# BrandonHanx/TextReID

Hardware: AMD Instinct MI355X
Metric: image-text pairs/sec (train), CLIP-RN50 + BiGRU MoCo step, bs128/GPU (higher is better)
Workload: dtype f32; 1 GPU; configs[1]: CLIP-RN50 + GRU, bs128/GPU, 384x128 images, 64-token captions, MoCo queue 8192, fp32, 1xMI355X; random-init weights, synthetic inputs resident in HBM; global_batch=128, parallelism=dp1, optimizer=Adam (fused multi-tensor), step_launch=eager launches, four streams (chosen by the probe over the recorded step)

## Files before the change

### textreid_amd/csrc/gemm_p16.hip

```cpp

#include <algorithm>
#include <mutex>
#include <type_traits>

#include "split_common.h"

namespace trid {

constexpr int P16_BK = 32;

constexpr int p16_lds_bytes(int BM, int BN, int NW, int STAGES) {
    const int st = STAGES * (BM + BN) * 128;
    return (NW == 12 && BM * BN * 4 > st) ? BM * BN * 4 : st;
}

template <int N>
__device__ __forceinline__ void wait_vmcnt() {
    asm volatile("s_waitcnt vmcnt(%0)" ::"n"(N) : "memory");
}

__device__ __forceinline__ void dma16(const __amdgpu_buffer_rsrc_t& rs, uint4* lds_base, unsigned voffset, unsigned soffset) {
    typedef __attribute__((address_space(3))) void* lds_ptr;
    __builtin_amdgcn_raw_ptr_buffer_load_lds(rs, (lds_ptr)lds_base, 16, voffset, soffset, 0, 0);
}
// ... 622 lines not shown
            if (bnb) {
                b_mu = *reinterpret_cast<const float4*>(bb.mean + col);
                b_is = *reinterpret_cast<const float4*>(bb.invstd + col);
                b_sc = *reinterpret_cast<const float4*>(bb.scale + col);
                b_sh = *reinterpret_cast<const float4*>(bb.shift + col);
            }
#pragma unroll
            for (int ps = 0; ps < BM / RG; ++ps) {
                const int rl = ps * RG + rg, row = m0 + rl;
                if (row >= p.M || col >= p.N) continue;
                float4 v = *reinterpret_cast<const float4*>(Ct + rl * BN + 4 * c4);
                const long long at = (long long)row * p.ldc + col;
                float4 yv = make_float4(0.f, 0.f, 0.f, 0.f);
                if (bnb) yv = *reinterpret_cast<const float4*>(bb.y + (long long)row * p.N + col);
                if (!pre) {
                    v.x += bv4.x; v.y += bv4.y; v.z += bv4.z; v.w += bv4.w;
                    if (p.accumulate) {
                        float4 u;
                        if (p.c_fmt == 2) {
                            const uint2 ub = *reinterpret_cast<const uint2*>(Cb + at);
                            u = make_float4(__builtin_bit_cast(float, ub.x << 16), __builtin_bit_cast(float, ub.x & 0xffff0000u),
                                            __builtin_bit_cast(float, ub.y << 16), __builtin_bit_cast(float, ub.y & 0xffff0000u));
                        } else {
                            u = *reinterpret_cast<const float4*>(C + at);
                        }
                        if (p.cmask != nullptr) {
                            const long long qi = at >> 2;
                            const ulonglong2* mq = reinterpret_cast<const ulonglong2*>(p.cmask + (qi >> 6) * 4);
                            const ulonglong2 m01 = mq[0], m23 = mq[1];
                            const int bit = (int)(qi & 63);
                            u.x = ((m01.x >> bit) & 1ull) ? u.x : 0.f; u.y = ((m01.y >> bit) & 1ull) ? u.y : 0.f;
                            u.z = ((m23.x >> bit) & 1ull) ? u.z : 0.f; u.w = ((m23.y >> bit) & 1ull) ? u.w : 0.f;
                        }
                        v.x += u.x; v.y += u.y; v.z += u.z; v.w += u.w;
                    }
                    if (p.res != nullptr) {
                        const float4 rr = *reinterpret_cast<const float4*>(p.res + (long long)row * p.ldres + col);
                        v.x += rr.x; v.y += rr.y; v.z += rr.z; v.w += rr.w;
                    }
                    if (p.relu) { v.x = fmaxf(v.x, 0.f); v.y = fmaxf(v.y, 0.f); v.z = fmaxf(v.z, 0.f); v.w = fmaxf(v.w, 0.f); }
                }
                if (p.c_fmt == 2) *reinterpret_cast<uint2*>(Cb + at) = make_uint2(cvt_pk_bf16(v.x, v.y), cvt_pk_bf16(v.z, v.w));
                else *reinterpret_cast<float4*>(C + at) = v;
                if (bnb) {
                    const float4 xh = make_float4((yv.x - b_mu.x) * b_is.x, (yv.y - b_mu.y) * b_is.y, (yv.z - b_mu.z) * b_is.z, (yv.w - b_mu.w) * b_is.w);
                    float4 g = v;
                    if (bb.relu == 1) {
                        g.x = fmaf(yv.x, b_sc.x, b_sh.x) > 0.f ? g.x : 0.f; g.y = fmaf(yv.y, b_sc.y, b_sh.y) > 0.f ? g.y : 0.f;
                        g.z = fmaf(yv.z, b_sc.z, b_sh.z) > 0.f ? g.z : 0.f; g.w = fmaf(yv.w, b_sc.w, b_sh.w) > 0.f ? g.w : 0.f;
                    } else if (bb.relu == 2) {
                        const long long qi = ((long long)row * p.N + col) >> 2;
                        const ulonglong2* mq = reinterpret_cast<const ulonglong2*>(bb.mask + (qi >> 6) * 4);
                        const ulonglong2 m01 = mq[0], m23 = mq[1];
                        const int bit = (int)(qi & 63);
                        g.x = ((m01.x >> bit) & 1ull) ? g.x : 0.f; g.y = ((m01.y >> bit) & 1ull) ? g.y : 0.f;
                        g.z = ((m23.x >> bit) & 1ull) ? g.z : 0.f; g.w = ((m23.y >> bit) & 1ull) ? g.w : 0.f;
                    }
                    b_s1.x += g.x; b_s1.y += g.y; b_s1.z += g.z; b_s1.w += g.w;
                    b_s2.x = fmaf(g.x, xh.x, b_s2.x); b_s2.y = fmaf(g.y, xh.y, b_s2.y); b_s2.z = fmaf(g.z, xh.z, b_s2.z); b_s2.w = fmaf(g.w, xh.w, b_s2.w);
                    b_mg.x = fmaxf(b_mg.x, fabsf(g.x)); b_mg.y = fmaxf(b_mg.y, fabsf(g.y)); b_mg.z = fmaxf(b_mg.z, fabsf(g.z)); b_mg.w = fmaxf(b_mg.w, fabsf(g.w));
                    b_mx.x = fmaxf(b_mx.x, fabsf(xh.x)); b_mx.y = fmaxf(b_mx.y, fabsf(xh.y)); b_mx.z = fmaxf(b_mx.z, fabsf(xh.z)); b_mx.w = fmaxf(b_mx.w, fabsf(xh.w));
                }
            }
            if (bb.y != nullptr) {
                __syncthreads();
                float* redf = reinterpret_cast<float*>(smem);
                float* mine = redf + (rg * C4 + c4) * 16;
                *reinterpret_cast<float4*>(mine) = b_s1;
                *reinterpret_cast<float4*>(mine + 4) = b_s2;
                *reinterpret_cast<float4*>(mine + 8) = b_mg;
                *reinterpret_cast<float4*>(mine + 12) = b_mx;
                __syncthreads();
                if (tid < C4 && n0 + 4 * tid < p.N) {
                    float4 s1 = make_float4(0.f, 0.f, 0.f, 0.f), s2 = s1, mg = s1, mx = s1;
                    for (int r = 0; r < RG; ++r) {
                        const float* src = redf + (r * C4 + tid) * 16;
                        const float4 a = *reinterpret_cast<const float4*>(src), b = *reinterpret_cast<const float4*>(src + 4);
                        const float4 c = *reinterpret_cast<const float4*>(src + 8), d = *reinterpret_cast<const float4*>(src + 12);
                        s1.x += a.x; s1.y += a.y; s1.z += a.z; s1.w += a.w;
                        s2.x += b.x; s2.y += b.y; s2.z += b.z; s2.w += b.w;
                        mg.x = fmaxf(mg.x, c.x); mg.y = fmaxf(mg.y, c.y); mg.z = fmaxf(mg.z, c.z); mg.w = fmaxf(mg.w, c.w);
                        mx.x = fmaxf(mx.x, d.x); mx.y = fmaxf(mx.y, d.y); mx.z = fmaxf(mx.z, d.z); mx.w = fmaxf(mx.w, d.w);
                    }
                    const int CQ = p.N >> 2, CW = CQ < 256 ? CQ : 256, S = CQ / CW;
                    const int q = (n0 >> 2) + tid;
                    const long long e = bn_bwd_partial_index(mb * S + q / CW, q % CW, p.mblocks * S, CQ);
                    *reinterpret_cast<float4*>(bb.ws + e) = s1;
                    *reinterpret_cast<float4*>(bb.ws + e + 4) = s2;
                    *reinterpret_cast<float4*>(bb.ws2 + e) = mg;
                    *reinterpret_cast<float4*>(bb.ws2 + e + 4) = mx;
                }
            }
            return;
        }
    }
#pragma unroll
    for (int j = 0; j < TN; ++j) {
        const int col = col_base + 32 * j;
        const float bv = (bias != nullptr && col < p.N) ? bias[col] : 0.f;
#pragma unroll
        for (int i = 0; i < TM; ++i) {
            float oldv[16];
            if (p.accumulate) {
#pragma unroll
                for (int r = 0; r < 16; ++r) {
                    const int row = row_base + i * 32 + (r & 3) + 8 * (r >> 2);
                    const long long at = (long long)row * p.ldc + col;
                    if (row < p.M && col < p.N) {
                        oldv[r] = p.c_fmt == 2 ? __builtin_bit_cast(float, (unsigned)Cb[at] << 16) : C[at];
                        if (p.cmask != nullptr && !((p.cmask[((at >> 2) >> 6) * 4 + (at & 3)] >> ((at >> 2) & 63)) & 1ull)) oldv[r] = 0.f;
                    } else {
                        oldv[r] = 0.f;
                    }
                }
            }
#pragma unroll
            for (int r = 0; r < 16; ++r) {
                const int row = row_base + i * 32 + (r & 3) + 8 * (r >> 2);
                float v = p.alpha * unscale * acc[i][j][r] + bv;
                if (p.accumulate) v += oldv[r];
                if (p.res != nullptr && row < p.M && col < p.N) v += p.res[(long long)row * p.ldres + col];
                if (p.relu) v = fmaxf(v, 0.f);
                if (row < p.M && col < p.N) {
                    const long long at = (long long)row * p.ldc + col;
                    if (p.c_fmt == 2) Cb[at] = (unsigned short)(cvt_pk_bf16(v, 0.f) & 0xffffu);
                    else C[at] = v;
                }
                acc[i][j][r] = p.c_fmt == 2 ? __builtin_bit_cast(float, cvt_pk_bf16(v, 0.f) << 16) : v;
            }
        }
    }

    if (p.stats != nullptr) emit_stats();
}

typedef __fp16 h4v __attribute__((__vector_size__(4 * sizeof(__fp16))));

__device__ __forceinline__ f16x8 tr_frag(const char* lds_addr) {
    typedef __attribute__((address_space(3))) h4v* lp;
    const h4v lo = __builtin_amdgcn_ds_read_tr16_b64_v4f16((lp)(lds_addr));
    const h4v hi = __builtin_amdgcn_ds_read_tr16_b64_v4f16((lp)(lds_addr + 512));
    f16x8 r;
    r[0] = lo[0]; r[1] = lo[1]; r[2] = lo[2]; r[3] = lo[3];
    r[4] = hi[0]; r[5] = hi[1]; r[6] = hi[2]; r[7] = hi[3];
    return r;
}

template <int BMODE, int BM, int STAGES, int PL, int SP = 0>
__global__ __launch_bounds__(512, 4) void gemm_p16_wgrad_kernel(GemmParams p) {
    constexpr int BN = 128, NW = 8, WN = 4, WM = 2;
    constexpr int GC = PL == 2 ? 32 : 64;
    constexpr int PBK = PL == 2 ? 32 : 64;
    constexpr int EB = PL == 2 ? 4 : 2;
    constexpr int CPG = PBK / 8;
    constexpr int TM = BM / (32 * WM);
    constexpr int A_CH = (BM / GC) * CPG, B_CH = (BN / GC) * CPG;
    constexpr int A_PW = (A_CH + NW - 1) / NW, B_PW = B_CH / NW;
    constexpr int PER_TILE = A_PW + B_PW;
    constexpr int GBYTES = PBK * 128;
    constexpr int A_BYTES = (BM / GC) * GBYTES, STAGE_BYTES = A_BYTES + (BN / GC) * GBYTES;
    extern __shared__ __attribute__((aligned(16))) uint4 smem[];
    char* const sbase = reinterpret_cast<char*>(smem);

    const float scaleA = (PL == 2 && p.a_amax != nullptr) ? f16_scale_of(*p.a_amax) : 1.f;
    const float scaleB = (PL == 2 && p.b_amax != nullptr) ? f16_scale_of(*p.b_amax) : 1.f;
    const int tid = threadIdx.x;
    const int lane = tid & 63;
    const int wave = __builtin_amdgcn_readfirstlane(tid >> 6);
    const int wm = wave / WN, wn = wave % WN;

    const uint32_t nwg = (uint32_t)p.mblocks * (uint32_t)p.nblocks;
    uint32_t lid;
    int sz;
    if (p.xcd_split) {
        const uint32_t slot = blockIdx.x >> 3;
        sz = (int)((slot / nwg) * 8 + (blockIdx.x & 7));
        lid = slot % nwg;
        if (sz >= p.splits) return;
    } else {
        lid = xcd_remap(blockIdx.x, nwg);
        sz = blockIdx.z;
    }
    const int mb = lid / p.nblocks, nb = lid % p.nblocks;
    const int m0 = mb * BM, n0 = nb * BN;
    const int k_begin = sz * p.k_chunk;
    const int k_end = min(p.K, k_begin + p.k_chunk);
    const int nk = (k_end - k_begin + PBK - 1) / PBK;
    float* __restrict__ C = p.C + (long long)sz * p.sSplit;

    constexpr unsigned OOB = 0x80000000u;
    const char* A = reinterpret_cast<const char*>(p.A);
    const char* Bp = reinterpret_cast<const char*>(p.B);
    const long long a_ld = p.lda * EB, b_ld = (BMODE == B_CONV ? (long long)p.Cin : p.ldb) * EB;
    const __amdgpu_buffer_rsrc_t rsA = __builtin_amdgcn_make_buffer_rsrc((void*)A, 0, (unsigned)((long long)p.K * a_ld), 0x00020000);
    const char* b_base = (BMODE == B_CONV) ? Bp - (long long)(p.W + 1) * b_ld : Bp;
    const long long b_rows = (BMODE == B_CONV) ? (long long)p.K + 2 * p.W + 2 : p.K;
    const __amdgpu_buffer_rsrc_t rsB = __builtin_amdgcn_make_buffer_rsrc((void*)b_base, 0, (unsigned)(b_rows * b_ld), 0x00020000);

    unsigned voA[A_PW], voB[B_PW];
    int b_pp[B_PW], b_dy[B_PW], b_dx[B_PW];
#pragma unroll
    for (int j = 0; j < A_PW; ++j) {
        const int c = j * NW + wave;
        const int gi = c / CPG, pp = 8 * (c % CPG) + (lane >> 3);
        const int s = (lane & 7) ^ (((pp >> 1) & 1) << 2);
        voA[j] = (c < A_CH && m0 + GC * gi < p.M) ? (unsigned)((long long)pp * a_ld + (m0 + GC * gi) * EB + 16 * s) : OOB;
    }
#pragma unroll
    for (int j = 0; j < B_PW; ++j) {
        const int c = j * NW + wave;
        const int gi = c / CPG, pp = 8 * (c % CPG) + (lane >> 3);
        const int s = (lane & 7) ^ (((pp >> 1) & 1) << 2);
        const int col = n0 + GC * gi;
        b_pp[j] = pp;
        b_dy[j] = b_dx[j] = 0;
        if (BMODE == B_CONV) {
            const int tap = col / p.Cin, c0 = col - tap * p.Cin;
            b_dy[j] = tap / 3 - 1;
            b_dx[j] = tap % 3 - 1;
            voB[j] = col < p.N ? (unsigned)((long long)(pp + (b_dy[j] + 1) * p.W + (b_dx[j] + 1)) * b_ld + c0 * EB + 16 * s) : OOB;
        } else {
            voB[j] = col < p.N ? (unsigned)((long long)pp * b_ld + col * EB + 16 * s) : OOB;
        }
    }

    auto issue = [&](int kt, int stage) {
        char* sA = sbase + stage * STAGE_BYTES;
        char* sB = sA + A_BYTES;
        const int k0 = k_begin + kt * PBK;
        const unsigned soA = (unsigned)((long long)k0 * a_ld), soB = (unsigned)((long long)k0 * b_ld);
#pragma unroll
        for (int j = 0; j < A_PW; ++j) {
            const int c = j * NW + wave;
            if (A_CH % NW != 0 && c >= A_CH) break;
            const unsigned vo = (k0 + 8 * (c % CPG) + (lane >> 3) < k_end) ? voA[j] : OOB;
            dma16(rsA, reinterpret_cast<uint4*>(sA + c * 1024), vo, soA);
        }
#pragma unroll
        for (int j = 0; j < B_PW; ++j) {
            const int c = j * NW + wave;
            unsigned vo = voB[j];
            const int m = k0 + b_pp[j];
            bool ok = m < k_end;
            if (BMODE == B_CONV) {
                const uint32_t q = fdiv((uint32_t)m, p.fdW);
                const int x = m - (int)q * p.W;
                const uint32_t b = fdiv(q, p.fdH);
                const int y = (int)q - (int)b * p.H;
                const int yy = y + b_dy[j], xx = x + b_dx[j];
                ok = ok && yy >= 0 && yy < p.H && xx >= 0 && xx < p.W;
            }
            dma16(rsB, reinterpret_cast<uint4*>(sB + c * 1024), ok ? vo : OOB, soB);
        }
    };

    v16f acc[TM];
#pragma unroll
    for (int i = 0; i < TM; ++i)
#pragma unroll
        for (int r = 0; r < 16; ++r) acc[i][r] = 0.f;

    const int h = (lane >> 4) & 1, r4 = (lane & 15) >> 2, c8 = lane & 3, kh = lane >> 5;
    const int swz = (r4 >> 1) << 2;
    auto frag_off = [&](int sub, int pl, int ks) {
        const int gi = (32 * sub) / GC;
        const int slot = PL == 2 ? (pl * 4 + h * 2 + (c8 >> 1)) : (((sub & 1) * 2 + h) * 2 + (c8 >> 1));
        return gi * GBYTES + (16 * ks + 8 * kh + r4) * 128 + ((slot ^ swz) << 4) + 8 * (c8 & 1);
    };

    auto compute = [&](int stage) {
        const char* sA = sbase + stage * STAGE_BYTES;
        const char* sB = sA + A_BYTES;
        if constexpr (PL == 1) {
#pragma unroll
            for (int ks = 0; ks < 4; ++ks) {
                bf16x8 a[TM], b;
#pragma unroll
                for (int i = 0; i < TM; ++i) a[i] = __builtin_bit_cast(bf16x8, tr_frag(sA + frag_off(wm * TM + i, 0, ks)));
                b = __builtin_bit_cast(bf16x8, tr_frag(sB + frag_off(wn, 0, ks)));
#pragma unroll
                for (int i = 0; i < TM; ++i) acc[i] = __builtin_amdgcn_mfma_f32_32x32x16_bf16(a[i], b, acc[i], 0, 0, 0);
            }
        } else {
#pragma unroll
            for (int ks = 0; ks < 2; ++ks) {
                f16x8 a[2][TM], b[2];
#pragma unroll
                for (int pl = 0; pl < 2; ++pl) {
#pragma unroll
                    for (int i = 0; i < TM; ++i) a[pl][i] = tr_frag(sA + frag_off(wm * TM + i, pl, ks));
                    b[pl] = tr_frag(sB + frag_off(wn, pl, ks));
                }
#pragma unroll
                for (int i = 0; i < TM; ++i) acc[i] = __builtin_amdgcn_mfma_f32_32x32x16_f16(a[0][i], b[1], acc[i], 0, 0, 0);
#pragma unroll
                for (int i = 0; i < TM; ++i) acc[i] = __builtin_amdgcn_mfma_f32_32x32x16_f16(a[1][i], b[0], acc[i], 0, 0, 0);
#pragma unroll
                for (int i = 0; i < TM; ++i) acc[i] = __builtin_amdgcn_mfma_f32_32x32x16_f16(a[0][i], b[0], acc[i], 0, 0, 0);
            }
        }
    };

    const bool wave_live = (m0 + wm * (32 * TM) < p.M) && (n0 + wn * 32 < p.N);
    if constexpr (SP != 0) {
        static_assert(STAGES == 2 && PL == 2, "software pipeline: two stages, P16 operands");
        const v4i_t rsA_s = raw_rsrc(A, (unsigned)((long long)p.K * a_ld)), rsB_s = raw_rsrc(b_base, (unsigned)(b_rows * b_ld));
        const unsigned smem_base = (unsigned)(uintptr_t)(__attribute__((address_space(3))) void*)smem;
        unsigned nvA[A_PW], nvB[B_PW], n_soA = 0, n_soB = 0;
        auto prep = [&](int kt) {
            const int k0 = k_begin + kt * PBK;
            n_soA = (unsigned)((long long)k0 * a_ld);
            n_soB = (unsigned)((long long)k0 * b_ld);
#pragma unroll
            for (int j = 0; j < A_PW; ++j) {
                const int c = j * NW + wave;
                nvA[j] = (k0 + 8 * (c % CPG) + (lane >> 3) < k_end) ? voA[j] : OOB;
            }
#pragma unroll
            for (int j = 0; j < B_PW; ++j) {
                const int m = k0 + b_pp[j];
                bool ok = m < k_end;
                if (BMODE == B_CONV) {
                    const uint32_t q = fdiv((uint32_t)m, p.fdW);
                    const int x = m - (int)q * p.W;
                    const uint32_t b = fdiv(q, p.fdH);
                    const int y = (int)q - (int)b * p.H;
                    const int yy = y + b_dy[j], xx = x + b_dx[j];
                    ok = ok && yy >= 0 && yy < p.H && xx >= 0 && xx < p.W;
                }
                nvB[j] = ok ? voB[j] : OOB;
            }
        };
        auto fire = [&](int stage) {
            const unsigned sA = smem_base + (unsigned)(stage * STAGE_BYTES), sB = sA + A_BYTES;
#pragma unroll
            for (int j = 0; j < A_PW; ++j) {
                const int c = j * NW + wave;
                if (A_CH % NW != 0 && c >= A_CH) break;
                dma16_asm(rsA_s, sA + (unsigned)c * 1024u, nvA[j], n_soA);
            }
#pragma unroll
            for (int j = 0; j < B_PW; ++j) dma16_asm(rsB_s, sB + (unsigned)(j * NW + wave) * 1024u, nvB[j], n_soB);
        };
        f16x8 f0a[2][TM], f0b[2], f1a[2][TM], f1b[2];
        auto rd = [&](int stage, int ks, f16x8 (&fa)[2][TM], f16x8 (&fb)[2]) {
            const char* sA = sbase + stage * STAGE_BYTES;
            const char* sB = sA + A_BYTES;
#pragma unroll
            for (int pl = 0; pl < 2; ++pl) {
#pragma unroll
                for (int i = 0; i < TM; ++i) fa[pl][i] = tr_frag(sA + frag_off(wm * TM + i, pl, ks));
                fb[pl] = tr_frag(sB + frag_off(wn, pl, ks));
            }
        };
        auto mm = [&](const f16x8 (&fa)[2][TM], const f16x8 (&fb)[2]) {
#pragma unroll
            for (int i = 0; i < TM; ++i) acc[i] = __builtin_amdgcn_mfma_f32_32x32x16_f16(fa[0][i], fb[1], acc[i], 0, 0, 0);
#pragma unroll
            for (int i = 0; i < TM; ++i) acc[i] = __builtin_amdgcn_mfma_f32_32x32x16_f16(fa[1][i], fb[0], acc[i], 0, 0, 0);
#pragma unroll
            for (int i = 0; i < TM; ++i) acc[i] = __builtin_amdgcn_mfma_f32_32x32x16_f16(fa[0][i], fb[0], acc[i], 0, 0, 0);
        };
        auto tile = [&](int t, auto stage_c) {
            constexpr int stage = decltype(stage_c)::value;
            asm volatile("s_waitcnt vmcnt(0)" ::: "memory");
            __builtin_amdgcn_s_waitcnt(0x0070);
            __builtin_amdgcn_s_barrier();
            asm volatile("" ::: "memory");
            if (wave_live) rd(stage, 0, f0a, f0b);
            __builtin_amdgcn_sched_barrier(0);
            if (t + 1 < nk) fire(stage ^ 1);
            __builtin_amdgcn_sched_barrier(0);
            if (wave_live) {
                if (t > 0) mm(f1a, f1b);
                __builtin_amdgcn_sched_barrier(0);
                rd(stage, 1, f1a, f1b);
            }
            __builtin_amdgcn_sched_barrier(0);
            if (t + 2 < nk) prep(t + 2);
            if (wave_live) mm(f0a, f0b);
            __builtin_amdgcn_sched_barrier(0);
        };
        typedef std::integral_constant<int, 0> S0;
        typedef std::integral_constant<int, 1> S1;
        if (nk > 0) {
            prep(0);
            fire(0);
            if (nk > 1) prep(1);
            int t = 0;
            for (; t + 1 < nk; t += 2) {
                tile(t, S0());
                tile(t + 1, S1());
            }
            if (t < nk) tile(t, S0());
            if (wave_live) mm(f1a, f1b);
        }
    } else {
#pragma unroll
        for (int s = 0; s < STAGES - 1; ++s)
            if (s < nk) issue(s, s);
        int stage = 0, istage = (STAGES - 1) % STAGES;
        for (int t = 0; t < nk; ++t) {
            const int ahead = min(STAGES - 2, nk - 1 - t);
            if (STAGES >= 3 && ahead >= 1) wait_vmcnt<PER_TILE>();
            else wait_vmcnt<0>();
            __builtin_amdgcn_s_barrier();
            asm volatile("" ::: "memory");
            if (t + STAGES - 1 < nk) issue(t + STAGES - 1, istage);
            if (wave_live) compute(stage);
            stage = (stage + 1 == STAGES) ? 0 : stage + 1;
            istage = (istage + 1 == STAGES) ? 0 : istage + 1;
        }
    }

    const float f = p.alpha / (scaleA * scaleB);
    const int row_base = m0 + wm * (32 * TM) + 4 * kh;
    const int col = n0 + wn * 32 + (lane & 31);
#pragma unroll
    for (int i = 0; i < TM; ++i)
#pragma unroll
        for (int r = 0; r < 16; ++r) {
            const int row = row_base + i * 32 + (r & 3) + 8 * (r >> 2);
            if (row < p.M && col < p.N) C[(long long)row * p.ldc + col] = f * acc[i][r];
        }
}

__device__ __forceinline__ void pack8_store(uint4* __restrict__ out, long long row, int K, int kg, const float (&v)[8], float scale, int fmt) {
    if (fmt == 2) {
        out[row * (K / 8) + kg] = make_uint4(cvt_pk_bf16(v[0], v[1]), cvt_pk_bf16(v[2], v[3]), cvt_pk_bf16(v[4], v[5]), cvt_pk_bf16(v[6], v[7]));
        return;
    }
    unsigned h[4], l[4];
#pragma unroll
    for (int q = 0; q < 4; ++q) f16_split2(v[2 * q] * scale, v[2 * q + 1] * scale, h[q], l[q]);
    uint4* dst = out + row * (K / 4) + (kg >> 2) * 8 + (kg & 3);
    dst[0] = make_uint4(h[0], h[1], h[2], h[3]);
    dst[4] = make_uint4(l[0], l[1], l[2], l[3]);
}

__global__ __launch_bounds__(256) void p16_pack_kernel(const float* __restrict__ x, long long rows, int K, long long ldx,
                                                       const float* __restrict__ amax, uint4* __restrict__ out, int fmt) {
    const float scale = (fmt == 1 && amax != nullptr) ? f16_scale_of(*amax) : 1.f;
    const int K8 = K / 8;
    const long long total = rows * K8;
    for (long long idx = (long long)blockIdx.x * 256 + threadIdx.x; idx < total; idx += (long long)gridDim.x * 256) {
        const long long row = idx / K8;
        const int kg = (int)(idx - row * K8);
        const float4 u = *reinterpret_cast<const float4*>(x + row * ldx + 8 * kg);
        const float4 v = *reinterpret_cast<const float4*>(x + row * ldx + 8 * kg + 4);
        const float x8[8] = {u.x, u.y, u.z, u.w, v.x, v.y, v.z, v.w};
        pack8_store(out, row, K, kg, x8, scale, fmt);
    }
}

__global__ __launch_bounds__(256) void p16_unpack_kernel(const uint4* __restrict__ in, long long rows, int K,
                                                         const float* __restrict__ amax, float* __restrict__ out) {
    const float inv = 1.f / (amax != nullptr ? f16_scale_of(*amax) : 1.f);
    const int K8 = K / 8;
    const long long total = rows * K8;
    for (long long idx = (long long)blockIdx.x * 256 + threadIdx.x; idx < total; idx += (long long)gridDim.x * 256) {
        const long long row = idx / K8;
        const int kg = (int)(idx - row * K8);
        const uint4* src = in + row * (K / 4) + (kg >> 2) * 8 + (kg & 3);
        const uint4 h = src[0], l = src[4];
        const unsigned hw[4] = {h.x, h.y, h.z, h.w}, lw[4] = {l.x, l.y, l.z, l.w};
        float v[8];
#pragma unroll
        for (int q = 0; q < 4; ++q) {
            const f16x2 a = __builtin_bit_cast(f16x2, hw[q]), b = __builtin_bit_cast(f16x2, lw[q]);
            v[2 * q] = ((float)a.x + (float)b.x) * inv;
            v[2 * q + 1] = ((float)a.y + (float)b.y) * inv;
        }
        float* dst = out + row * K + 8 * kg;
        *reinterpret_cast<float4*>(dst) = make_float4(v[0], v[1], v[2], v[3]);
        *reinterpret_cast<float4*>(dst + 4) = make_float4(v[4], v[5], v[6], v[7]);
    }
}

__global__ __launch_bounds__(256) void p16_pack_wt_kernel(const float* __restrict__ w, int N, int T, int C, int flip,
                                                          const float* __restrict__ amax, uint4* __restrict__ out) {
    const float scale = amax != nullptr ? f16_scale_of(*amax) : 1.f;
    const int K = T * N, K8 = K / 8;
    const long long total = (long long)C * K8;
    for (long long idx = (long long)blockIdx.x * 256 + threadIdx.x; idx < total; idx += (long long)gridDim.x * 256) {
        const int kg = (int)(idx / C);
        const int c = (int)(idx - (long long)kg * C);
        const int k0 = 8 * kg;
        const int tp = k0 / N, n0 = k0 - tp * N;
        const int t = flip ? T - 1 - tp : tp;
        float v[8];
#pragma unroll
        for (int i = 0; i < 8; ++i) v[i] = w[((long long)(n0 + i) * T + t) * C + c] * scale;
        unsigned h[4], l[4];
#pragma unroll
        for (int q = 0; q < 4; ++q) f16_split2(v[2 * q], v[2 * q + 1], h[q], l[q]);
        uint4* dst = out + (long long)c * (K / 4) + (kg >> 2) * 8 + (kg & 3);
        dst[0] = make_uint4(h[0], h[1], h[2], h[3]);
        dst[4] = make_uint4(l[0], l[1], l[2], l[3]);
    }
}

__global__ __launch_bounds__(256) void p16_pack_multi_kernel(const long long* __restrict__ table, const float* __restrict__ amax,
                                                             int transposed, int fmt) {
    const long long* e = table + 6 * (long long)blockIdx.y;
    const float* __restrict__ w = reinterpret_cast<const float*>(e[0]);
    uint4* __restrict__ out = reinterpret_cast<uint4*>(e[1]);
    const int N = (int)e[2], T = (int)e[3], C = (int)e[4];
    const float scale = fmt == 1 ? f16_scale_of(amax[e[5]]) : 1.f;
    if (!transposed) {
        const int K = T * C, K8 = K / 8;
        const long long total = (long long)N * K8;
        for (long long idx = (long long)blockIdx.x * 256 + threadIdx.x; idx < total; idx += (long long)gridDim.x * 256) {
            const long long row = idx / K8;
            const int kg = (int)(idx - row * K8);
            const float4 u = *reinterpret_cast<const float4*>(w + row * K + 8 * kg);
            const float4 v = *reinterpret_cast<const float4*>(w + row * K + 8 * kg + 4);
            const float x8[8] = {u.x, u.y, u.z, u.w, v.x, v.y, v.z, v.w};
            pack8_store(out, row, K, kg, x8, scale, fmt);
        }
    } else {
        const int K = T * N, K8 = K / 8;
        const long long total = (long long)C * K8;
        for (long long idx = (long long)blockIdx.x * 256 + threadIdx.x; idx < total; idx += (long long)gridDim.x * 256) {
            const int kg = (int)(idx / C);
            const int c = (int)(idx - (long long)kg * C);
            const int k0 = 8 * kg;
            const int tp = k0 / N, n0 = k0 - tp * N;
            const int t = T - 1 - tp;
            float v[8];
#pragma unroll
            for (int i = 0; i < 8; ++i) v[i] = w[((long long)(n0 + i) * T + t) * C + c];
            pack8_store(out, c, K, kg, v, scale, fmt);
        }
    }
}

template <int AMODE, int BM, int BN, int WM, int WN, int STAGES, int PL = 2, bool PP = false, int SP = 0>
static int launch_p16(GemmParams& p, hipStream_t stream) {
    p.mblocks = (p.M + BM - 1) / BM;
    p.nblocks = (p.N + BN - 1) / BN;
    dim3 grid((unsigned)(p.mblocks * p.nblocks), 1, (unsigned)(p.batch * p.splits));
    static const size_t pad = getenv("TRID_GEMM_LDS_PAD") ? (size_t)atoi(getenv("TRID_GEMM_LDS_PAD")) * 1024 : 0;
    const size_t lds = std::max((size_t)p16_lds_bytes(BM, BN, WM * WN, STAGES), pad);
    static std::once_flag once;
    static hipError_t attr_err = hipSuccess;
    std::call_once(once, [lds] {
        if (lds > 48 * 1024)
            attr_err = hipFuncSetAttribute((const void*)gemm_p16_kernel<AMODE, BM, BN, WM, WN, STAGES, PL, PP, SP>,
                                           hipFuncAttributeMaxDynamicSharedMemorySize, (int)lds);
    });
    if (attr_err != hipSuccess) {
        set_error("trid_gemm_p16: cannot reserve %zu B of LDS: %s", lds, hipGetErrorString(attr_err));
        return (int)attr_err;
    }
    hipLaunchKernelGGL((gemm_p16_kernel<AMODE, BM, BN, WM, WN, STAGES, PL, PP, SP>), grid, dim3(WM * WN * 64), lds, stream, p);
    return check_launch("trid_gemm_p16");
}

static bool tile192_rule(int M, int N) {
    static const int env = getenv("TRID_P16_TILE192") ? atoi(getenv("TRID_P16_TILE192")) : 0;
    if (!env || M % 192 != 0 || N % 128 != 0) return false;
    const long long t128 = (long long)((M + 127) / 128) * (N / 128), t192 = (long long)(M / 192) * (N / 128);
    return t128 > 256 && t128 < 512 && t192 % 256 == 0;
}

template <int AMODE>
static int pick_p16(GemmParams& p, int variant, int planes, hipStream_t stream) {
    if (planes == 1) {
        if (p.N <= 64) return launch_p16<AMODE, 128, 64, 2, 2, 3, 1>(p, stream);
        return launch_p16<AMODE, 128, 128, 2, 4, 2, 1>(p, stream);
    }
    if (p.N <= 32) return launch_p16<AMODE, 256, 32, 4, 1, 3>(p, stream);
    if (p.N <= 64) return launch_p16<AMODE, 128, 64, 2, 2, 3>(p, stream);
    static const int def_env = getenv("TRID_P16_DEFAULT_VARIANT") ? atoi(getenv("TRID_P16_DEFAULT_VARIANT")) : 12;
    if (variant < 0 && p.stats != nullptr && tile192_rule(p.M, p.N)) variant = 15;
    const bool tile8 = variant == 3 || variant == 10 || variant == 12 || variant == 14;
    if (variant < 0 || ((p.c_fmt == 1 || p.bb.y != nullptr) && !tile8)) variant = def_env;
    switch (variant) {
        case 1: return launch_p16<AMODE, 128, 128, 2, 2, 3>(p, stream);
        case 2: return launch_p16<AMODE, 256, 128, 4, 2, 3>(p, stream);
        case 3: return launch_p16<AMODE, 128, 128, 2, 4, 2>(p, stream);
        case 4: return launch_p16<AMODE, 256, 128, 4, 2, 2>(p, stream);
        case 5: return launch_p16<AMODE, 128, 128, 2, 4, 3>(p, stream);
        case 8: return launch_p16<AMODE, 128, 64, 2, 2, 2>(p, stream);
        case 9: return launch_p16<AMODE, 96, 128, 3, 2, 2>(p, stream);
        case 6: return launch_p16<AMODE, 128, 128, 2, 4, 2, 2, true>(p, stream);
        case 7: return launch_p16<AMODE, 256, 128, 4, 2, 2, 2, true>(p, stream);
        case 10: return launch_p16<AMODE, 128, 128, 2, 4, 2, 2, false, 1>(p, stream);
        case 11: return launch_p16<AMODE, 128, 128, 2, 2, 2, 2, false, 1>(p, stream);
        case 12: return launch_p16<AMODE, 128, 128, 2, 4, 2, 2, false, 2>(p, stream);
        case 13: return launch_p16<AMODE, 128, 128, 2, 2, 2, 2, false, 2>(p, stream);
        case 15: return launch_p16<AMODE, 192, 128, 3, 4, 2, 2, false, 2>(p, stream);
        case 16: return launch_p16<AMODE, 192, 128, 3, 4, 2, 2, false, 1>(p, stream);
        case 14: return launch_p16<AMODE, 128, 128, 2, 4, 2, 2, false, 6>(p, stream);
        default: return launch_p16<AMODE, 128, 128, 2, 2, 2>(p, stream);
    }
}

}

using namespace trid;

extern "C" int trid_p16_pack_f32(const float* x, long long rows, int K, long long ldx, const float* amax, void* out, int fmt,
                                 void* stream) {
    TRID_REQUIRE(x && out && rows > 0 && K > 0 && K % 32 == 0 && ldx % 4 == 0 && aligned16(x) && aligned16(out) && (fmt == 1 || fmt == 2),
                 "trid_p16_pack_f32: needs K %% 32 == 0, 16-byte aligned rows and fmt 1 / 2 (K=%d)", K);
    hipLaunchKernelGGL(p16_pack_kernel, dim3(grid_for(rows * (K / 8), 256, 8192)), dim3(256), 0, (hipStream_t)stream, x, rows, K,
                       ldx, amax, (uint4*)out, fmt);
    return check_launch("trid_p16_pack_f32");
}

extern "C" int trid_p16_unpack_f32(const void* in, long long rows, int K, const float* amax, float* out, void* stream) {
    TRID_REQUIRE(in && out && rows > 0 && K > 0 && K % 32 == 0 && aligned16(in) && aligned16(out), "trid_p16_unpack_f32: bad arguments");
    hipLaunchKernelGGL(p16_unpack_kernel, dim3(grid_for(rows * (K / 8), 256, 8192)), dim3(256), 0, (hipStream_t)stream,
                       (const uint4*)in, rows, K, amax, out);
    return check_launch("trid_p16_unpack_f32");
}

extern "C" int trid_p16_pack_wt_f32(const float* w, int N, int T, int C, int flip, const float* amax, void* out, void* stream) {
    TRID_REQUIRE(w && out && N > 0 && T > 0 && C > 0 && N % 8 == 0 && (T * N) % 32 == 0 && aligned16(out),
                 "trid_p16_pack_wt_f32: needs N %% 8 == 0 and T*N %% 32 == 0 (N=%d T=%d)", N, T);
    hipLaunchKernelGGL(p16_pack_wt_kernel, dim3(grid_for((long long)C * (T * N / 8), 256, 8192)), dim3(256), 0, (hipStream_t)stream,
                       w, N, T, C, flip, amax, (uint4*)out);
    return check_launch("trid_p16_pack_wt_f32");
}

template <int BMODE, int BM, int PL, int SP = 0>
static int launch_p16_wgrad(GemmParams& p, hipStream_t stream) {
    constexpr int STAGES = 2;
    p.mblocks = (p.M + BM - 1) / BM;
    p.nblocks = (p.N + 127) / 128;
    static const int xcd_env = getenv("TRID_WGRAD_XCD") ? atoi(getenv("TRID_WGRAD_XCD")) : 1;
    p.xcd_split = (xcd_env && p.splits >= 8) ? 1 : 0;
    dim3 grid((unsigned)(p.mblocks * p.nblocks), 1, (unsigned)p.splits);
    if (p.xcd_split) grid = dim3((unsigned)(p.mblocks * p.nblocks) * 8u * (unsigned)((p.splits + 7) / 8), 1, 1);
    static const size_t pad = getenv("TRID_WGRAD_LDS_PAD") ? (size_t)atoi(getenv("TRID_WGRAD_LDS_PAD")) * 1024 : 0;
    const size_t lds = std::max((size_t)STAGES * ((BM / 32) + 4) * 4096, pad);
    static std::once_flag once;
    static hipError_t attr_err = hipSuccess;
    std::call_once(once, [lds] {
        if (lds > 48 * 1024)
            attr_err = hipFuncSetAttribute((const void*)gemm_p16_wgrad_kernel<BMODE, BM, STAGES, PL, SP>, hipFuncAttributeMaxDynamicSharedMemorySize, (int)lds);
    });
    if (attr_err != hipSuccess) {
        set_error("trid_gemm_p16_wgrad: cannot reserve %zu B of LDS: %s", lds, hipGetErrorString(attr_err));
        return (int)attr_err;
    }
    hipLaunchKernelGGL((gemm_p16_wgrad_kernel<BMODE, BM, STAGES, PL, SP>), grid, dim3(512), lds, stream, p);
    return check_launch("trid_gemm_p16_wgrad");
}

extern "C" int trid_gemm_p16_wgrad(const trid_gemm_desc* d, void* stream_) {
    hipStream_t stream = (hipStream_t)stream_;
    TRID_REQUIRE(d != nullptr && d->A && d->B && d->C, "trid_gemm_p16_wgrad: null operand");
    TRID_REQUIRE(d->a_mode == A_MC && (d->b_mode == B_NC || d->b_mode == B_CONV), "trid_gemm_p16_wgrad: loader modes A_MC x B_NC / B_CONV only");
    const int planes = d->precision == 1 ? 1 : 2;
    const int gc = planes == 1 ? 64 : 32;
    TRID_REQUIRE(d->M > 0 && d->N > 0 && d->K > 0 && d->M % gc == 0 && d->N % gc == 0 && d->lda % gc == 0,
                 "trid_gemm_p16_wgrad: M, N and the row pitches must be multiples of %d (M=%d N=%d)", gc, d->M, d->N);
    TRID_REQUIRE(d->batch == 1 && d->splits >= 1 && !d->accumulate && !d->bias && !d->residual && !d->relu && !d->stats,
                 "trid_gemm_p16_wgrad: plain or split-K output only");
    TRID_REQUIRE(aligned16(d->A) && aligned16(d->B) && aligned16(d->C), "trid_gemm_p16_wgrad: operands must be 16-byte aligned");
    GemmParams p;
    memset(&p, 0, sizeof(p));
    p.A = d->A; p.B = d->B; p.C = d->C;
    p.M = d->M; p.N = d->N; p.K = d->K;
    p.lda = d->lda; p.ldb = d->ldb; p.ldc = d->ldc;
    p.batch = 1; p.splits = d->splits;
    p.alpha = d->alpha;
    p.H = d->H; p.W = d->W; p.Cin = d->Cin;
    p.a_amax = d->a_amax; p.b_amax = d->b_amax;
    if (d->b_mode == B_CONV) {
        TRID_REQUIRE(d->H > 0 && d->W > 0 && d->Cin > 0 && d->Cin % gc == 0 && d->N == 9 * d->Cin && d->K % (d->H * d->W) == 0,
                     "trid_gemm_p16_wgrad: B_CONV needs Cin %% %d == 0, N == 9*Cin, K a multiple of H*W", gc);
        p.fdW = make_fastdiv((uint32_t)d->W);
        p.fdH = make_fastdiv((uint32_t)d->H);
        TRID_REQUIRE((long long)(d->K + 2 * d->W + 2) * d->Cin * 4 < (1ll << 31), "trid_gemm_p16_wgrad: operands must stay below 2 GB");
    } else {
        TRID_REQUIRE(d->ldb % 32 == 0 && (long long)d->K * d->ldb * 4 < (1ll << 31), "trid_gemm_p16_wgrad: ldb %% 32 and B below 2 GB");
    }
    TRID_REQUIRE((long long)d->K * d->lda * 4 < (1ll << 31), "trid_gemm_p16_wgrad: operands must stay below 2 GB");
    const int pbk = planes == 1 ? 64 : 32;
    int kc = (d->K + d->splits - 1) / d->splits;
    kc = (kc + pbk - 1) / pbk * pbk;
    p.k_chunk = kc;
    p.sSplit = d->strideSplit;
    if (planes == 1) {
        if (d->b_mode == B_CONV) return d->M <= 64 ? launch_p16_wgrad<B_CONV, 64, 1>(p, stream) : launch_p16_wgrad<B_CONV, 128, 1>(p, stream);
        return d->M <= 64 ? launch_p16_wgrad<B_NC, 64, 1>(p, stream) : launch_p16_wgrad<B_NC, 128, 1>(p, stream);
    }
    static const int sp_env = getenv("TRID_WGRAD_SP") ? atoi(getenv("TRID_WGRAD_SP")) : 1;
    if (sp_env && d->M > 64) return d->b_mode == B_CONV ? launch_p16_wgrad<B_CONV, 128, 2, 1>(p, stream) : launch_p16_wgrad<B_NC, 128, 2, 1>(p, stream);
    if (d->b_mode == B_CONV) return d->M <= 64 ? launch_p16_wgrad<B_CONV, 64, 2>(p, stream) : launch_p16_wgrad<B_CONV, 128, 2>(p, stream);
    return d->M <= 64 ? launch_p16_wgrad<B_NC, 64, 2>(p, stream) : launch_p16_wgrad<B_NC, 128, 2>(p, stream);
}

extern "C" int trid_p16_pack_multi_f32(const long long* table, const float* amax, int n_tensors, int transposed, int fmt, void* stream) {
    TRID_REQUIRE(table && (amax || fmt == 2) && n_tensors > 0 && (fmt == 1 || fmt == 2), "trid_p16_pack_multi_f32: bad arguments");
    hipLaunchKernelGGL(p16_pack_multi_kernel, dim3(64, (unsigned)n_tensors), dim3(256), 0, (hipStream_t)stream, table, amax, transposed, fmt);
    return check_launch("trid_p16_pack_multi_f32");
}

extern "C" int trid_gemm_p16_rows(int M, int N, int precision, int variant) {
    if (precision == 1 || N <= 64) return 128;
    if (variant < 0) return tile192_rule(M, N) ? 192 : 128;
    return variant == 9 ? 96 : ((variant == 15 || variant == 16) ? 192 : 128);
}

static int wide_env_ok() {
    static const int wide_env = getenv("TRID_GEMM_WIDE_EPILOGUE") ? atoi(getenv("TRID_GEMM_WIDE_EPILOGUE")) : 1;
    return wide_env;
}

extern "C" int trid_gemm_p16_bnb_ok(int M, int N) {
    const int CQ = N / 4;
    return (M > 0 && N > 0 && (N == 64 || N % 128 == 0) && (256 % CQ == 0 || CQ % 256 == 0) && (long long)M * N * 4 < (1ll << 31) && wide_env_ok()) ? 1 : 0;
}

extern "C" int trid_gemm_p16(const trid_gemm_desc* d, int variant, void* stream_) {
    hipStream_t stream = (hipStream_t)stream_;
    TRID_REQUIRE(d != nullptr && d->A && d->B && d->C, "trid_gemm_p16: null operand");
    const int planes = d->precision == 1 ? 1 : 2;
    const int bke = planes == 1 ? 64 : 32;
    TRID_REQUIRE(d->M > 0 && d->N > 0 && d->K > 0 && d->K % bke == 0, "trid_gemm_p16: K must be a positive multiple of %d (K=%d)", bke, d->K);
    TRID_REQUIRE((d->a_mode == A_KC || d->a_mode == A_CONV) && d->b_mode == B_KC, "trid_gemm_p16: loader modes A_KC / A_CONV x B_KC only");
    TRID_REQUIRE(aligned16(d->A) && aligned16(d->B) && aligned16(d->C), "trid_gemm_p16: operands must be 16-byte aligned");
    TRID_REQUIRE(d->batch >= 1 && d->splits >= 1, "trid_gemm_p16: batch/splits must be >= 1");
    TRID_REQUIRE(d->lda % 32 == 0 && d->ldb % 32 == 0, "trid_gemm_p16: row pitches must be multiples of 32 elements");
    TRID_REQUIRE(planes == 2 || d->N >= 64, "trid_gemm_p16: bf16 operands need N >= 64");
    GemmParams p;
    memset(&p, 0, sizeof(p));
    p.A = d->A; p.B = d->B; p.C = d->C;
    p.M = d->M; p.N = d->N; p.K = d->K;
    p.lda = d->lda; p.ldb = d->ldb; p.ldc = d->ldc;
    p.sA = d->strideA; p.sB = d->strideB; p.sC = d->strideC;
    p.batch = d->batch; p.splits = d->splits;
    p.alpha = d->alpha; p.accumulate = d->accumulate;
    p.bias = d->bias; p.sBias = d->strideBias; p.stats = d->stats;
    p.res = d->residual; p.ldres = d->ldres; p.relu = d->relu;
    p.H = d->H; p.W = d->W; p.Cin = d->Cin;
    p.a_amax = d->a_amax; p.b_amax = d->b_amax;
    p.stats_w = d->stats_minmax ? 4 : 2;
    p.c_fmt = d->c_format;
    p.cmask = reinterpret_cast<const unsigned long long*>(d->c_mask);
    p.colscale = d->col_scale; p.res16 = d->res_p16; p.res16_amax = d->res_amax;
    p.ev.coef = d->eval_coef; p.ev.tin = d->eval_tin; p.ev.tres = d->eval_tres;
    p.ev.out_bound = d->out_bound; p.ev.out_tmax = d->out_tmax;
    p.pool_w = d->eval_pool_w;
    p.bb.y = d->bnb_y; p.bb.mean = d->bnb_mean; p.bb.invstd = d->bnb_invstd; p.bb.scale = d->bnb_scale; p.bb.shift = d->bnb_shift;
    p.bb.ws = d->bnb_ws; p.bb.ws2 = d->bnb_ws2; p.bb.relu = d->bnb_relu;
    p.bb.mask = reinterpret_cast<const unsigned long long*>(d->bnb_mask);
    if (d->bnb_y != nullptr) {
        const int CQ = d->N / 4;
        TRID_REQUIRE(planes == 2 && d->c_format == 0 && d->batch == 1 && d->splits == 1 && d->ldc == d->N && (d->N == 64 || d->N % 128 == 0) && !d->stats &&
                     (256 % CQ == 0 || CQ % 256 == 0) && wide_env_ok(),
                     "trid_gemm_p16: the BatchNorm-backward sums (bnb_y) need P16 operands, fp32 C with ldc == N, N == 64 or N %% 128 == 0, batch == splits == 1, no stats (N=%d)", d->N);
        TRID_REQUIRE(d->bnb_relu >= 0 && d->bnb_relu <= 2 && (d->bnb_relu != 2 || (d->bnb_mask != nullptr && aligned16(d->bnb_mask))),
                     "trid_gemm_p16: bnb_relu must be 0, 1 or 2 (2: with the 16-byte aligned ReLU bit mask bnb_mask)");
        TRID_REQUIRE(d->bnb_mean && d->bnb_invstd && d->bnb_scale && d->bnb_shift && d->bnb_ws && d->bnb_ws2 && aligned16(d->bnb_y) && aligned16(d->bnb_mean) &&
                     aligned16(d->bnb_invstd) && aligned16(d->bnb_scale) && aligned16(d->bnb_shift) && aligned16(d->bnb_ws) && aligned16(d->bnb_ws2),
                     "trid_gemm_p16: the BatchNorm-backward sums need all of bnb_mean / invstd / scale / shift / ws / ws2, 16-byte aligned");
    }
    TRID_REQUIRE(p.cmask == nullptr || (d->accumulate && d->batch == 1 && d->splits == 1 && d->ldc == d->N && d->N % 4 == 0 && !d->stats),
                 "trid_gemm_p16: c_mask needs accumulate, batch == splits == 1, ldc == N, N %% 4 == 0");
    p.wide_epilogue = wide_env_ok();
    TRID_REQUIRE(p.c_fmt == 0 || ((p.c_fmt == 2 || p.c_fmt == 1) && d->batch == 1 && d->splits == 1),
                 "trid_gemm_p16: c_format must be 0, or 1 / 2 with batch == splits == 1");
    if (p.c_fmt == 1) {
        TRID_REQUIRE(planes == 2 && !d->accumulate && !d->stats && !d->residual && d->ldc == d->N && d->N % 32 == 0 && (long long)d->M * d->N * 4 < (1ll << 31),
                     "trid_gemm_p16: the eval epilogue (c_format 1) needs P16 operands, ldc == N, N %% 32 == 0, no accumulate / stats / fp32 residual (N=%d)", d->N);
        TRID_REQUIRE(d->eval_coef && d->eval_tin && (!d->res_p16 || (d->res_amax && d->eval_tres && aligned16(d->res_p16))) && (!d->col_scale || aligned16(d->col_scale)) &&
                     (!d->bias || aligned16(d->bias)), "trid_gemm_p16: the eval epilogue needs eval_coef / eval_tin (and res_amax / eval_tres with a residual), 16-byte aligned vectors");
        p.wide_epilogue = 1;
        if (d->eval_pool_w) {
            TRID_REQUIRE(d->a_mode == A_CONV && d->eval_pool_w == d->W && d->W % 2 == 0 && d->H % 2 == 0 && 128 % d->W == 0 && (128 / d->W) % 2 == 0 &&
                         (d->H * d->W) % 128 == 0 && d->N > 64 && !d->res_p16,
                         "trid_gemm_p16: the pooled eval epilogue needs a 3x3 convolution with W | 128, an even number of image rows per 128-row tile, H * W %% 128 == 0, N > 64, no residual (H=%d W=%d N=%d)", d->H, d->W, d->N);
        }
    } else {
        TRID_REQUIRE(!d->col_scale && !d->res_p16, "trid_gemm_p16: col_scale / res_p16 belong to the eval epilogue (c_format 1)");
    }
    if (d->a_mode == A_CONV) {
        TRID_REQUIRE(d->H > 0 && d->W > 0 && d->Cin > 0 && d->Cin % bke == 0 && d->K == 9 * d->Cin && d->M % (d->H * d->W) == 0 && d->splits == 1,
                     "trid_gemm_p16: A_CONV needs Cin %% %d == 0, K == 9*Cin, M a multiple of H*W, splits == 1", bke);
        p.fdW = make_fastdiv((uint32_t)d->W);
        p.fdH = make_fastdiv((uint32_t)d->H);
    }
    TRID_REQUIRE(!(d->stats && (d->splits != 1 || d->batch != 1)), "trid_gemm_p16: stats epilogue needs splits==1, batch==1");
    TRID_REQUIRE(!(d->splits > 1 && (d->accumulate || d->bias || d->residual || d->relu)), "trid_gemm_p16: split-K writes raw slabs");
    const long long a_bytes = (d->a_mode == A_CONV ? (long long)(d->M + 2 * d->W + 2) * d->Cin : (long long)d->M * d->lda) * 4;
    TRID_REQUIRE(a_bytes < (1ll << 31) && (long long)d->N * d->ldb * 4 < (1ll << 31), "trid_gemm_p16: operands must stay below 2 GB (31-bit buffer offsets)");
    int kc = (d->K + d->splits - 1) / d->splits;
    kc = (kc + bke - 1) / bke * bke;
    p.k_chunk = kc;
    p.sSplit = d->strideSplit;
    if (d->a_mode == A_CONV) return pick_p16<A_CONV>(p, variant, planes, stream);
    return pick_p16<A_KC>(p, variant, planes, stream);
}
```

Before: 3148 pairs/s.

## Add deeper software-pipelined wgrad GEMM variant with incremental conv coordinates

Adds a new SP=2 path for the two-plane wgrad GEMM. It splits each K tile into two LDS fragment reads and interleaves them with the previous tile's MFMAs and the next tile's DMA issue. Conv pixel coordinates are stepped incrementally instead of recomputed by division each tile, and the whole loop is specialized at compile time on wave liveness. This is now the default for M>64, with the aim of hiding LDS read latency and cutting index arithmetic. The cost is more fragment registers live at once, which could lower occupancy.

```diff
diff --git a/textreid_amd/csrc/gemm_p16.hip b/textreid_amd/csrc/gemm_p16.hip
--- a/textreid_amd/csrc/gemm_p16.hip
+++ b/textreid_amd/csrc/gemm_p16.hip
@@ -948,7 +948,126 @@
     };
 
     const bool wave_live = (m0 + wm * (32 * TM) < p.M) && (n0 + wn * 32 < p.N);
-    if constexpr (SP != 0) {
+    if constexpr (SP == 2) {
+        static_assert(STAGES == 2 && PL == 2, "software pipeline: two stages, P16 operands");
+        const v4i_t rsA_s = raw_rsrc(A, (unsigned)((long long)p.K * a_ld)), rsB_s = raw_rsrc(b_base, (unsigned)(b_rows * b_ld));
+        const unsigned smem_base = (unsigned)(uintptr_t)(__attribute__((address_space(3))) void*)smem;
+        unsigned nvA[A_PW], nvB[B_PW], n_soA = 0, n_soB = 0;
+        int n_k0 = k_begin;
+        constexpr int NPX = NW % CPG == 0 ? 1 : B_PW;
+        int px[NPX], py[NPX];
+        const int step_x = BMODE == B_CONV ? PBK % p.W : 0, step_y = BMODE == B_CONV ? (PBK / p.W) % p.H : 0;
+#pragma unroll
+        for (int j = 0; j < NPX; ++j) {
+            px[j] = py[j] = 0;
+            if (BMODE == B_CONV) {
+                const uint32_t m = (uint32_t)(k_begin + b_pp[j]);
+                const uint32_t q = fdiv(m, p.fdW);
+                px[j] = (int)(m - q * (uint32_t)p.W);
+                py[j] = (int)(q - fdiv(q, p.fdH) * (uint32_t)p.H);
+            }
+        }
+        auto prep = [&]() {
+            n_soA = (unsigned)((long long)n_k0 * a_ld);
+            n_soB = (unsigned)((long long)n_k0 * b_ld);
+#pragma unroll
+            for (int j = 0; j < A_PW; ++j) {
+                const int c = j * NW + wave;
+                nvA[j] = (n_k0 + 8 * (c % CPG) + (lane >> 3) < k_end) ? voA[j] : OOB;
+            }
+#pragma unroll
+            for (int j = 0; j < B_PW; ++j) {
+                const int jp = NPX == 1 ? 0 : j;
+                bool ok = n_k0 + b_pp[jp] < k_end;
+                if (BMODE == B_CONV)
+                    ok = ok && (unsigned)(py[jp] + b_dy[j]) < (unsigned)p.H && (unsigned)(px[jp] + b_dx[j]) < (unsigned)p.W;
+                nvB[j] = ok ? voB[j] : OOB;
+            }
+            if (BMODE == B_CONV) {
+#pragma unroll
+                for (int j = 0; j < NPX; ++j) {
+                    int x = px[j] + step_x, y = py[j] + step_y;
+                    if (x >= p.W) { x -= p.W; ++y; }
+                    if (y >= p.H) y -= p.H;
+                    px[j] = x;
+                    py[j] = y;
+                }
+            }
+            n_k0 += PBK;
+        };
+        auto fire = [&](int stage) {
+            const unsigned sA = smem_base + (unsigned)(stage * STAGE_BYTES), sB = sA + A_BYTES;
+#pragma unroll
+            for (int j = 0; j < A_PW; ++j) {
+                const int c = j * NW + wave;
+                if (A_CH % NW != 0 && c >= A_CH) break;
+                dma16_asm(rsA_s, sA + (unsigned)c * 1024u, nvA[j], n_soA);
+            }
+#pragma unroll
+            for (int j = 0; j < B_PW; ++j) dma16_asm(rsB_s, sB + (unsigned)(j * NW + wave) * 1024u, nvB[j], n_soB);
+        };
+        f16x8 f0a[2][TM], f0b[2], f1a[2][TM], f1b[2];
+        auto rd = [&](int stage, int ks, f16x8 (&fa)[2][TM], f16x8 (&fb)[2]) {
+            const char* sA = sbase + stage * STAGE_BYTES;
+            const char* sB = sA + A_BYTES;
+#pragma unroll
+            for (int pl = 0; pl < 2; ++pl) {
+#pragma unroll
+                for (int i = 0; i < TM; ++i) fa[pl][i] = tr_frag(sA + frag_off(wm * TM + i, pl, ks));
+                fb[pl] = tr_frag(sB + frag_off(wn, pl, ks));
+            }
+        };
+        auto mm = [&](const f16x8 (&fa)[2][TM], const f16x8 (&fb)[2]) {
+#pragma unroll
+            for (int i = 0; i < TM; ++i) acc[i] = __builtin_amdgcn_mfma_f32_32x32x16_f16(fa[0][i], fb[1], acc[i], 0, 0, 0);
+#pragma unroll
+            for (int i = 0; i < TM; ++i) acc[i] = __builtin_amdgcn_mfma_f32_32x32x16_f16(fa[1][i], fb[0], acc[i], 0, 0, 0);
+#pragma unroll
+            for (int i = 0; i < TM; ++i) acc[i] = __builtin_amdgcn_mfma_f32_32x32x16_f16(fa[0][i], fb[0], acc[i], 0, 0, 0);
+        };
+        typedef std::integral_constant<int, 0> S0;
+        typedef std::integral_constant<int, 1> S1;
+        typedef std::true_type Y;
+        typedef std::false_type N;
+        auto tile = [&](auto stage_c, auto live_c, auto prev_c, bool next) {
+            constexpr int stage = decltype(stage_c)::value;
+            constexpr bool live = decltype(live_c)::value, has_prev = decltype(prev_c)::value;
+            asm volatile("s_waitcnt vmcnt(0)" ::: "memory");
+            __builtin_amdgcn_s_waitcnt(0x0070);
+            __builtin_amdgcn_s_barrier();
+            asm volatile("" ::: "memory");
+            if constexpr (live) rd(stage, 0, f0a, f0b);
+            __builtin_amdgcn_sched_barrier(0);
+            if (next) fire(stage ^ 1);
+            __builtin_amdgcn_sched_barrier(0);
+            if constexpr (live) {
+                if constexpr (has_prev) mm(f1a, f1b);
+                __builtin_amdgcn_sched_barrier(0);
+                rd(stage, 1, f1a, f1b);
+            }
+            __builtin_amdgcn_sched_barrier(0);
+            prep();
+            if constexpr (live) mm(f0a, f0b);
+            __builtin_amdgcn_sched_barrier(0);
+        };
+        auto run = [&](auto live_c) {
+            prep();
+            fire(0);
+            prep();
+            tile(S0(), live_c, N(), 1 < nk);
+            int t = 1;
+            for (; t + 1 < nk; t += 2) {
+                tile(S1(), live_c, Y(), t + 1 < nk);
+                tile(S0(), live_c, Y(), t + 2 < nk);
+            }
+            if (t < nk) tile(S1(), live_c, Y(), false);
+            if constexpr (decltype(live_c)::value) mm(f1a, f1b);
+        };
+        if (nk > 0) {
+            if (wave_live) run(Y());
+            else run(N());
+        }
+    } else if constexpr (SP != 0) {
         static_assert(STAGES == 2 && PL == 2, "software pipeline: two stages, P16 operands");
         const v4i_t rsA_s = raw_rsrc(A, (unsigned)((long long)p.K * a_ld)), rsB_s = raw_rsrc(b_base, (unsigned)(b_rows * b_ld));
         const unsigned smem_base = (unsigned)(uintptr_t)(__attribute__((address_space(3))) void*)smem;
@@ -1335,8 +1454,9 @@
         if (d->b_mode == B_CONV) return d->M <= 64 ? launch_p16_wgrad<B_CONV, 64, 1>(p, stream) : launch_p16_wgrad<B_CONV, 128, 1>(p, stream);
         return d->M <= 64 ? launch_p16_wgrad<B_NC, 64, 1>(p, stream) : launch_p16_wgrad<B_NC, 128, 1>(p, stream);
     }
-    static const int sp_env = getenv("TRID_WGRAD_SP") ? atoi(getenv("TRID_WGRAD_SP")) : 1;
-    if (sp_env && d->M > 64) return d->b_mode == B_CONV ? launch_p16_wgrad<B_CONV, 128, 2, 1>(p, stream) : launch_p16_wgrad<B_NC, 128, 2, 1>(p, stream);
+    static const int sp_env = getenv("TRID_WGRAD_SP") ? atoi(getenv("TRID_WGRAD_SP")) : 2;
+    if (sp_env >= 2 && d->M > 64) return d->b_mode == B_CONV ? launch_p16_wgrad<B_CONV, 128, 2, 2>(p, stream) : launch_p16_wgrad<B_NC, 128, 2, 2>(p, stream);
+    if (sp_env == 1 && d->M > 64) return d->b_mode == B_CONV ? launch_p16_wgrad<B_CONV, 128, 2, 1>(p, stream) : launch_p16_wgrad<B_NC, 128, 2, 1>(p, stream);
     if (d->b_mode == B_CONV) return d->M <= 64 ? launch_p16_wgrad<B_CONV, 64, 2>(p, stream) : launch_p16_wgrad<B_CONV, 128, 2>(p, stream);
     return d->M <= 64 ? launch_p16_wgrad<B_NC, 64, 2>(p, stream) : launch_p16_wgrad<B_NC, 128, 2>(p, stream);
 }
```

New measurement: 3146 pairs/s (median of 6 runs). Within noise of the previous version (-0.1%).
